# zendesk/min-tfs-client

Measured on AMD Instinct MI355X. Metric: predict_req_per_s, higher is better.
Workload: dtype fp32; 1 GPU; model=identity-echo[resnet50], global_batch=32, parallelism=dp1, pipeline=4, encoding=turbo, grpc_impl=native, copy_mode=1, streaming=auto, transport=unix, servers_per_rank=1, gpu=True

## Files before the change

### min_tfs_client_amd/ops/csrc/grpc_transport.cpp

```cpp
#include <pybind11/eval.h>
#include <pybind11/functional.h>
#include <pybind11/pybind11.h>
#include <pybind11/stl.h>
#include <torch/extension.h>

#include <c10/hip/HIPCachingAllocator.h>
#include <c10/hip/HIPGuard.h>
#include <c10/hip/HIPStream.h>

#include <algorithm>
#include <atomic>
#include <chrono>
#include <condition_variable>
#include <cstring>
#include <deque>
#include <map>
#include <memory>
#include <mutex>
#include <set>
#include <string>
#include <thread>
#include <unordered_map>
#include <vector>

#include "h2core.h"
#include "hpack.h"
#include "sharded.h"
#include "staging.h"
#include "wire.h"

namespace py = pybind11;

namespace {

using h2::Buf;
using h2::Conn;
using h2::ConnError;
using h2::FrameHeader;

struct WireRegion {
  size_t offset;
  size_t nbytes;
  uintptr_t ptr;
  bool device;
};

void write_message_with_regions(Conn& conn, uint32_t stream,
                                const uint8_t* buf, size_t len,
                                const std::vector<WireRegion>& regions,
                                bool end_stream) {
  h2::DataMessageWriter w(conn, stream, len, end_stream);
  size_t pos = 0;
  for (const auto& r : regions) {
    if (r.offset < pos || r.nbytes > len || r.offset > len - r.nbytes)
      throw ConnError("bad streaming region");
    if (r.offset > pos) w.write(buf + pos, r.offset - pos);
    if (!r.device) {
      w.write(reinterpret_cast<const uint8_t*>(r.ptr), r.nbytes);
    } else {
      mi355x_staging::Lease lease;
      lease.ctx->d2h(reinterpret_cast<const void*>(r.ptr), r.nbytes,
                     [&w](const void* chunk, size_t n) {
                       w.write(static_cast<const uint8_t*>(chunk), n);
                     });
    }
    pos = r.offset + r.nbytes;
  }
  if (pos < len) w.write(buf + pos, len - pos);
  w.finish();
}

bool extract_streaming_reply(py::handle result,
                             std::unique_ptr<py::buffer_info>* info,
                             const uint8_t** buf, size_t* len,
                             std::vector<WireRegion>* regions) {
  if (!py::hasattr(result, "_wire_regions")) return false;
  py::object buffer = result.attr("buffer");
  *info = std::make_unique<py::buffer_info>(py::buffer(buffer).request());
  *buf = static_cast<const uint8_t*>((*info)->ptr);
  *len = size_t((*info)->size) * size_t((*info)->itemsize);
  for (auto item : result.attr("_wire_regions")) {
    auto t = py::reinterpret_borrow<py::tuple>(item);
    regions->push_back(WireRegion{
        t[0].cast<size_t>(), t[1].cast<size_t>(),
        uintptr_t(t[2].cast<uint64_t>()), t[3].cast<bool>()});
  }
  return true;
}

struct RpcCallError : std::runtime_error {
  int code;
  RpcCallError(int code_, const std::string& msg)
      : std::runtime_error(msg), code(code_) {}
};

constexpr int GRPC_OK = 0;
constexpr int GRPC_CANCELLED = 1;
constexpr int GRPC_UNKNOWN = 2;
constexpr int GRPC_INVALID_ARGUMENT = 3;
constexpr int GRPC_DEADLINE_EXCEEDED = 4;
constexpr int GRPC_RESOURCE_EXHAUSTED = 8;
constexpr int GRPC_UNIMPLEMENTED = 12;
constexpr int GRPC_INTERNAL = 13;
constexpr int GRPC_UNAVAILABLE = 14;

struct OwnedBuf {
  Buf buf;
  explicit OwnedBuf(Buf&& b) : buf(std::move(b)) {}
};

class PinnedPool {
 public:
  static PinnedPool& instance() {
    static PinnedPool* pool = new PinnedPool();
    return *pool;
  }

  static constexpr size_t kMinPinned = 1u << 20;
  static constexpr size_t kMaxCached = 512u << 20;

  bool available() {
    int state = state_.load(std::memory_order_acquire);
    if (state == 0) {
      int n = 0;
      bool ok = hipGetDeviceCount(&n) == hipSuccess && n > 0;
      state = ok ? 1 : -1;
      state_.store(state, std::memory_order_release);
    }
    return state > 0;
  }

  uint8_t* get(size_t n, size_t* cap_out) {
    if (n < kMinPinned || !available()) return nullptr;
    size_t cap = size_class(n);
    {
      std::lock_guard<std::mutex> lk(mu_);
      auto& fl = free_[cap];
      if (!fl.empty()) {
        uint8_t* p = fl.back();
        fl.pop_back();
        cached_ -= cap;
        *cap_out = cap;
        return p;
      }
    }
    void* p = nullptr;
    if (hipHostMalloc(&p, cap) != hipSuccess) return nullptr;
    *cap_out = cap;
    return static_cast<uint8_t*>(p);
  }

  void put(uint8_t* p, size_t cap) {
    {
      std::lock_guard<std::mutex> lk(mu_);
      if (cached_ + cap <= kMaxCached) {
        free_[cap].push_back(p);
        cached_ += cap;
        return;
      }
    }
    (void)hipHostFree(p);
  }

  static void deleter(void* ctx, uint8_t* p, size_t cap) {
    static_cast<PinnedPool*>(ctx)->put(p, cap);
  }

 private:
  static size_t size_class(size_t n) {
    size_t cap = kMinPinned;
    while (cap < n) cap <<= 1;
    return cap;
  }
  std::atomic<int> state_{0};
  std::mutex mu_;
  std::map<size_t, std::vector<uint8_t*>> free_;
  size_t cached_ = 0;
};


inline bool tf_dtype_to_scalar(int dt, at::ScalarType* st) {
  switch (dt) {
    case 1: *st = at::kFloat; return true;
    case 2: *st = at::kDouble; return true;
    case 3: *st = at::kInt; return true;
    case 4: *st = at::kByte; return true;
    case 5: *st = at::kShort; return true;
    case 6: *st = at::kChar; return true;
    case 8: *st = at::kComplexFloat; return true;
    case 9: *st = at::kLong; return true;
    case 10: *st = at::kBool; return true;
    case 14: *st = at::kBFloat16; return true;
    case 17: *st = at::kUInt16; return true;
    case 18: *st = at::kComplexDouble; return true;
    case 19: *st = at::kHalf; return true;
    case 22: *st = at::kUInt32; return true;
    case 23: *st = at::kUInt64; return true;
    default: return false;
  }
}


inline void record_consumer_stream(
    std::vector<std::pair<std::string, at::Tensor>>& outs, int device) {
  if (outs.empty()) return;
  auto cur = c10::hip::getCurrentHIPStream(
      static_cast<c10::DeviceIndex>(device));
  for (auto& kv : outs)
    c10::hip::HIPCachingAllocator::recordStream(
        kv.second.storage().data_ptr(), cur);
}

struct MsgAssemblyFwd;

class ProspectStreams {
 public:
  static ProspectStreams& instance() {
    static ProspectStreams* p = new ProspectStreams();
    return *p;
  }

  static constexpr int kPerDevice = 4;

  hipStream_t get(int device) {
    std::lock_guard<std::mutex> lk(mu_);
    auto it = per_dev_.find(device);
    if (it == per_dev_.end()) {
      std::vector<hipStream_t> v;
      if (hipSetDevice(device) == hipSuccess) {
        for (int i = 0; i < kPerDevice; ++i) {
          hipStream_t s = nullptr;
          if (hipStreamCreateWithFlags(&s, hipStreamNonBlocking) !=
              hipSuccess)
            break;
          v.push_back(s);
        }
      }
      it = per_dev_.emplace(device, std::move(v)).first;
    }
    if (it->second.empty()) return nullptr;
    return it->second[rr_++ % it->second.size()];
  }

 private:
  std::mutex mu_;
  std::unordered_map<int, std::vector<hipStream_t>> per_dev_;
  size_t rr_ = 0;
};

struct DeviceParse {
  bool enabled = false;
  bool failed = false;
  bool done = false;
  int device = 0;
  hipStream_t stream = nullptr;
  int spec_field = 2;
  int map_field = 1;
  std::string spec_name, spec_signature, spec_label;
  int64_t spec_version = -1;
  std::vector<std::string> out_filter;
  std::function<bool(const std::string&)> skip_model;
  size_t pos = 0;
  int state = 0;
  size_t entry_end = 0, tp_end = 0;
  std::string cur_name;
  int cur_dtype = 0;
  std::vector<int64_t> cur_shape;
  bool cur_has_tensor = false;
  at::Tensor cur_tensor;
  bool in_content = false;
  size_t content_off = 0, content_len = 0, content_copied = 0;
  bool copies_issued = false;
  std::vector<std::pair<std::string, at::Tensor>> outs;

  static constexpr size_t kCopyBatch = 1u << 20;

  void fail() {
    failed = true;
    in_content = false;
  }

  void quiesce() {
    if (copies_issued && stream != nullptr) {
      (void)hipStreamSynchronize(stream);
      copies_issued = false;
    }
  }

  DeviceParse() = default;
  DeviceParse(const DeviceParse&) = delete;
  DeviceParse& operator=(const DeviceParse&) = delete;
  DeviceParse(DeviceParse&& o) noexcept { *this = std::move(o); }
  DeviceParse& operator=(DeviceParse&& o) noexcept {
    if (this != &o) {
      quiesce();
      enabled = o.enabled; failed = o.failed; done = o.done;
      device = o.device; stream = o.stream;
      spec_field = o.spec_field; map_field = o.map_field;
      spec_name = std::move(o.spec_name);
      spec_signature = std::move(o.spec_signature);
      spec_label = std::move(o.spec_label);
      spec_version = o.spec_version;
      out_filter = std::move(o.out_filter);
      skip_model = std::move(o.skip_model);
      pos = o.pos; state = o.state;
      entry_end = o.entry_end; tp_end = o.tp_end;
      cur_name = std::move(o.cur_name);
      cur_dtype = o.cur_dtype;
      cur_shape = std::move(o.cur_shape);
      cur_has_tensor = o.cur_has_tensor;
      cur_tensor = std::move(o.cur_tensor);
      in_content = o.in_content;
      content_off = o.content_off;
      content_len = o.content_len;
      content_copied = o.content_copied;
      copies_issued = o.copies_issued;
      outs = std::move(o.outs);
      o.copies_issued = false;
      o.enabled = false;
      o.stream = nullptr;
    }
    return *this;
  }
  ~DeviceParse() { quiesce(); }
};

struct MsgAssembly {
  uint8_t prefix[5];
  size_t prefix_have = 0;
  Buf msg;
  size_t msg_have = 0;
  bool have_len = false;

  void feed_from_socket(int fd, size_t n) {
    while (n > 0) {
      if (prefix_have < 5) {
        size_t take = 5 - prefix_have < n ? 5 - prefix_have : n;
        h2::read_full(fd, prefix + prefix_have, take);
        prefix_have += take;
        n -= take;
        if (prefix_have == 5) {
          if (prefix[0] != 0)
            throw RpcCallError(GRPC_UNIMPLEMENTED,
                               "compressed gRPC messages not supported");
          uint32_t len = h2::be32(prefix + 1);
          if (len > (1u << 30))
            throw RpcCallError(
                GRPC_RESOURCE_EXHAUSTED,
                "received message larger than max (" +
                    std::to_string(len) + " vs 1073741824)");
          size_t cap = 0;
          auto& pool = PinnedPool::instance();
          uint8_t* pinned = pool.get(len, &cap);
          if (pinned != nullptr)
            msg.adopt(pinned, cap, &PinnedPool::deleter, &pool);
          else
            msg.alloc(len);
          msg.len = len;
          have_len = true;
        }
        continue;
      }
      if (!have_len || msg_have + n > msg.len)
        throw ConnError("DATA overruns gRPC message length");
      h2::read_full(fd, msg.p + msg_have, n);
      msg_have += n;
      n = 0;
    }
  }

  bool complete() const { return have_len && msg_have == msg.len; }
};

inline void device_parse_advance(DeviceParse& dp, MsgAssembly& body) {
  if (!dp.enabled || dp.failed || dp.done) return;
  if (!body.have_len) return;
  if (dp.pos == 0 && dp.outs.empty() && !dp.in_content) {
    if (body.msg.deleter == nullptr || body.msg.len < (1u << 20)) {
      dp.enabled = false;
      return;
    }
  }
  const uint8_t* base = body.msg.p;
  const size_t watermark = body.msg_have;
  const size_t total = body.msg.len;

  auto issue_copies = [&]() -> bool {
    size_t span_end = dp.content_off + dp.content_len;
    size_t have_end = watermark < span_end ? watermark : span_end;
    size_t done_abs = dp.content_off + dp.content_copied;
    if (have_end > done_abs) {
      size_t n = have_end - done_abs;
      bool flush = have_end == span_end || body.complete();
      if (n >= DeviceParse::kCopyBatch || flush) {
        if (hipSetDevice(dp.device) != hipSuccess) { dp.fail(); return false; }
        char* dst = static_cast<char*>(dp.cur_tensor.data_ptr())
                    + dp.content_copied;
        if (hipMemcpyAsync(dst, base + done_abs, n, hipMemcpyHostToDevice,
                           dp.stream) != hipSuccess) {
          dp.fail();
          return false;
        }
        dp.copies_issued = true;
        dp.content_copied += n;
      }
    }
    return dp.content_copied == dp.content_len;
  };

  try {
    while (true) {
      if (dp.in_content) {
        if (!issue_copies()) return;
        if (dp.failed) return;
        dp.in_content = false;
        dp.pos = dp.content_off + dp.content_len;
        dp.cur_has_tensor = true;
      }
      tfswire::Cursor c{base + dp.pos, base + watermark};
      const uint8_t* step_start = c.p;
      try {
        if (dp.state == 0) {
          if (dp.pos == total) {
            dp.done = true;
            return;
          }
          int wt = 0;
          int f = c.read_tag(&wt);
          if (f == dp.spec_field && wt == tfswire::WT_LEN) {
            tfswire::Cursor spec = c.read_len_delim();
            while (!spec.done()) {
              int swt = 0;
              int sf = spec.read_tag(&swt);
              if (sf == 1 && swt == tfswire::WT_LEN) {
                tfswire::Cursor v = spec.read_len_delim();
                dp.spec_name.assign(reinterpret_cast<const char*>(v.p),
                                    size_t(v.end - v.p));
              } else if (sf == 2 && swt == tfswire::WT_LEN) {
                tfswire::Cursor v = spec.read_len_delim();
                while (!v.done()) {
                  int vwt = 0;
                  int vf = v.read_tag(&vwt);
                  if (vf == 1 && vwt == tfswire::WT_VARINT)
                    dp.spec_version = int64_t(v.read_varint());
                  else
                    v.skip(vwt);
                }
              } else if (sf == 3 && swt == tfswire::WT_LEN) {
                tfswire::Cursor v = spec.read_len_delim();
                dp.spec_signature.assign(
                    reinterpret_cast<const char*>(v.p),
                    size_t(v.end - v.p));
              } else if (sf == 4 && swt == tfswire::WT_LEN) {
                tfswire::Cursor v = spec.read_len_delim();
                dp.spec_label.assign(reinterpret_cast<const char*>(v.p),
                                     size_t(v.end - v.p));
              } else {
                spec.skip(swt);
              }
            }
            if (dp.skip_model && dp.skip_model(dp.spec_name)) {
              dp.enabled = false;
              return;
            }
            dp.pos = size_t(c.p - base);
          } else if (f == dp.map_field && wt == tfswire::WT_LEN) {
            uint64_t len = c.read_varint();
            size_t body_off = size_t(c.p - base);
            if (body_off + len > total) { dp.fail(); return; }
            dp.entry_end = body_off + len;
            dp.pos = body_off;
            dp.state = 1;
          } else if (dp.spec_field == 1 && f == 3 &&
                     wt == tfswire::WT_LEN) {
            tfswire::Cursor v = c.read_len_delim();
            dp.out_filter.emplace_back(
                reinterpret_cast<const char*>(v.p), size_t(v.end - v.p));
            dp.pos = size_t(c.p - base);
          } else {
            dp.fail();
            return;
          }
        } else if (dp.state == 1) {
          int wt = 0;
          int f = c.read_tag(&wt);
          if (f != 1 || wt != tfswire::WT_LEN) { dp.fail(); return; }
          tfswire::Cursor key = c.read_len_delim();
          dp.cur_name.assign(reinterpret_cast<const char*>(key.p),
                             size_t(key.end - key.p));
          f = c.read_tag(&wt);
          if (f != 2 || wt != tfswire::WT_LEN) { dp.fail(); return; }
          uint64_t len = c.read_varint();
          size_t body_off = size_t(c.p - base);
          if (body_off + len > dp.entry_end) { dp.fail(); return; }
          dp.tp_end = body_off + len;
          dp.pos = body_off;
          dp.state = 2;
          dp.cur_dtype = 0;
          dp.cur_shape.clear();
          dp.cur_has_tensor = false;
          dp.cur_tensor = at::Tensor();
        } else {
          if (dp.pos == dp.tp_end) {
            if (!dp.cur_has_tensor) {
              int64_t numel = 1;
              for (int64_t d : dp.cur_shape) numel *= d;
              at::ScalarType st;
              if (numel == 0 && tf_dtype_to_scalar(dp.cur_dtype, &st)) {
                c10::hip::HIPStreamGuard g(c10::hip::getStreamFromExternal(
                    dp.stream, static_cast<c10::DeviceIndex>(dp.device)));
                dp.cur_tensor = at::empty(
                    dp.cur_shape, at::TensorOptions().dtype(st).device(
                                      at::kCUDA, dp.device));
                dp.cur_has_tensor = true;
              } else {
                dp.fail();
                return;
              }
            }
            dp.outs.emplace_back(dp.cur_name, dp.cur_tensor);
            dp.cur_tensor = at::Tensor();
            if (dp.pos != dp.entry_end) { dp.fail(); return; }
            dp.state = 0;
            continue;
          }
          int wt = 0;
          int f = c.read_tag(&wt);
          if (f == 1 && wt == tfswire::WT_VARINT) {
            dp.cur_dtype = int(c.read_varint());
          } else if (f == 2 && wt == tfswire::WT_LEN) {
            tfswire::Cursor sh = c.read_len_delim();
            dp.cur_shape.clear();
            while (!sh.done()) {
              int swt = 0;
              int sf = sh.read_tag(&swt);
              if (sf == 2 && swt == tfswire::WT_LEN) {
                tfswire::Cursor dim = sh.read_len_delim();
                int64_t size = 0;
                while (!dim.done()) {
                  int dwt = 0;
                  int df = dim.read_tag(&dwt);
                  if (df == 1 && dwt == tfswire::WT_VARINT)
                    size = int64_t(dim.read_varint());
                  else
                    dim.skip(dwt);
                }
                dp.cur_shape.push_back(size);
              } else if (sf == 3) {
                dp.fail();
                return;
              } else {
                sh.skip(swt);
              }
            }
          } else if (f == 3 && wt == tfswire::WT_VARINT) {
            (void)c.read_varint();
          } else if (f == 4 && wt == tfswire::WT_LEN) {
            uint64_t len = c.read_varint();
            size_t off = size_t(c.p - base);
            if (off + len > dp.tp_end) { dp.fail(); return; }
            at::ScalarType st;
            if (!tf_dtype_to_scalar(dp.cur_dtype, &st)) { dp.fail(); return; }
            int64_t numel = 1;
            for (int64_t d : dp.cur_shape) numel *= d;
            size_t esize = at::elementSize(st);
            if (uint64_t(numel) * esize != len) { dp.fail(); return; }
            {
              c10::hip::HIPStreamGuard g(c10::hip::getStreamFromExternal(
                  dp.stream, static_cast<c10::DeviceIndex>(dp.device)));
              dp.cur_tensor = at::empty(
                  dp.cur_shape,
                  at::TensorOptions().dtype(st).device(at::kCUDA,
                                                       dp.device));
            }
            dp.content_off = off;
            dp.content_len = size_t(len);
            dp.content_copied = 0;
            dp.in_content = true;
            dp.pos = off;
            continue;
          } else {
            dp.fail();
            return;
          }
          dp.pos = size_t(c.p - base);
        }
      } catch (const std::exception&) {
        (void)step_start;
        if (body.complete()) dp.fail();
        return;
      }
    }
  } catch (...) {
    dp.fail();
  }
}

struct HeaderBlock {
  std::string block;
  bool end_stream = false;
  bool done = false;
};

inline void read_headers_fragment(int fd, const FrameHeader& fh,
                                  std::string* out) {
  uint32_t len = fh.length;
  uint8_t pad = 0;
  if (fh.flags & h2::FL_PADDED) {
    h2::read_full(fd, &pad, 1);
    if (len < 1u + pad) throw ConnError("bad padding");
    len -= 1;
  }
  if (fh.flags & h2::FL_PRIORITY) {
    uint8_t prio[5];
    if (len < 5) throw ConnError("bad priority");
    h2::read_full(fd, prio, 5);
    len -= 5;
  }
  len -= pad;
  size_t off = out->size();
  out->resize(off + len);
  h2::read_full(fd, reinterpret_cast<uint8_t*>(&(*out)[off]), len);
  if (pad) h2::discard(fd, pad);
}

inline const std::string* find_header(const std::vector<h2::Header>& hs,
                                      const char* name) {
  for (auto& h : hs)
    if (h.first == name) return &h.second;
  return nullptr;
}

inline std::string make_response_headers_block() {
  h2::HpackEncoder enc;
  std::string block;
  enc.add_indexed(&block, 8);
  enc.add_literal(&block, 31, "application/grpc");
  return block;
}

inline std::string make_trailers_block(int status, const std::string& msg) {
  h2::HpackEncoder enc;
  std::string block;
  enc.add_literal(&block, "grpc-status", std::to_string(status));
  if (!msg.empty())
    enc.add_literal(&block, "grpc-message", h2::percent_encode(msg));
  return block;
}

inline std::string make_trailers_only_block(int status,
                                            const std::string& msg) {
  h2::HpackEncoder enc;
  std::string block;
  enc.add_indexed(&block, 8);
  enc.add_literal(&block, 31, "application/grpc");
  enc.add_literal(&block, "grpc-status", std::to_string(status));
  if (!msg.empty())
    enc.add_literal(&block, "grpc-message", h2::percent_encode(msg));
  return block;
}

inline bool echo_eligible(const tfswire::ParsedPredict& req,
                          const std::map<std::string, std::set<int64_t>>&
                              models) {
  if (!req.output_filter.empty()) return false;
  auto it = models.find(req.model_spec.name);
  if (it == models.end()) return false;
  if (req.model_spec.version >= 0 &&
      it->second.find(req.model_spec.version) == it->second.end())
    return false;
  if (!req.model_spec.version_label.empty()) return false;
  for (auto& t : req.tensors)
    if (t.content == nullptr) return false;
  return true;
}

struct EchoResponse {
  Buf skeleton;
  std::vector<WireRegion> regions;
};

inline EchoResponse build_echo_response(const tfswire::ParsedPredict& req) {
  constexpr size_t kEchoMinRegion = 64 * 1024;
  std::vector<std::string> names;
  std::vector<tfswire::TensorMeta> metas;
  std::vector<const uint8_t*> payloads;
  names.reserve(req.tensors.size());
  for (auto& t : req.tensors) {
    std::string name = t.name;
    const std::string suffix = "_input";
    if (name.size() > suffix.size() &&
        name.compare(name.size() - suffix.size(), suffix.size(), suffix) ==
            0) {
      name = name.substr(0, name.size() - suffix.size()) + "_output";
    }
    names.push_back(std::move(name));
    metas.push_back({t.dtype, t.shape, t.content_bytes});
    payloads.push_back(t.content);
  }
  const std::string sig = req.model_spec.signature_name.empty()
                              ? "serving_default"
                              : req.model_spec.signature_name;
  auto plan = tfswire::plan_predict_message(false, req.model_spec.name,
                                            req.model_spec.version, sig,
                                            names, metas);
  EchoResponse r;
// ... 508 lines not shown
      std::lock_guard<std::mutex> lk(handler_mu_);
      parsed_path = parsed_paths_.count(t.path) != 0;
    }
    bool have_parse = parsed_path && t.dparse.enabled &&
                      !t.dparse.failed && t.dparse.done;
    t.dparse.quiesce();
    if (!Py_IsInitialized() || _Py_IsFinalizing()) {
      send_error_response(t, GRPC_UNAVAILABLE, "server shutting down");
      return;
    }
    int err_code = 0;
    std::string err_msg;
    py::object result;
    {
      py::gil_scoped_acquire gil;
      py::object fn;
      {
        std::lock_guard<std::mutex> lk(handler_mu_);
        auto it = py_handlers_.find(t.path);
        if (it != py_handlers_.end()) fn = it->second;
      }
      if (!fn) {
        err_code = GRPC_UNIMPLEMENTED;
        err_msg = "service method unregistered: " + t.path;
      } else
      try {
        py::memoryview view = py::memoryview::from_memory(
            t.msg.p, py::ssize_t(t.msg.len));
        if (parsed_path) {
          py::object spec = py::none();
          py::object outs = py::none();
          if (have_parse) {
            record_consumer_stream(t.dparse.outs, t.dparse.device);
            py::dict sd;
            sd["name"] = t.dparse.spec_name;
            sd["version"] = t.dparse.spec_version;
            sd["signature_name"] = t.dparse.spec_signature;
            sd["version_label"] = t.dparse.spec_label;
            py::list filt;
            for (auto& f2 : t.dparse.out_filter) filt.append(py::str(f2));
            sd["output_filter"] = filt;
            py::dict od;
            for (auto& kv : t.dparse.outs)
              od[py::str(kv.first)] = kv.second;
            spec = std::move(sd);
            outs = std::move(od);
          }
          result = fn(view, spec, outs);
        } else {
          result = fn(view);
        }
        t.dparse.outs.clear();
      } catch (py::error_already_set& e) {
        err_code = GRPC_UNKNOWN;
        try {
          py::object exc = e.value();
          if (py::hasattr(exc, "grpc_code"))
            err_code = exc.attr("grpc_code").cast<int>();
          if (py::hasattr(exc, "grpc_details"))
            err_msg = exc.attr("grpc_details").cast<std::string>();
          else
            err_msg = py::str(exc).cast<std::string>();
        } catch (...) {
          err_msg = "handler error";
        }
        e.restore();
        PyErr_Clear();
      }
    }
    if (err_code != 0) {
      send_error_response(t, err_code, err_msg);
      return;
    }
    std::unique_ptr<py::buffer_info> info;
    const uint8_t* ptr = nullptr;
    size_t len = 0;
    bool streaming = false;
    std::vector<WireRegion> regions;
    {
      py::gil_scoped_acquire gil;
      try {
        streaming = extract_streaming_reply(result, &info, &ptr, &len,
                                            &regions);
        if (!streaming) {
          info = std::make_unique<py::buffer_info>(
              py::buffer(result).request());
          ptr = static_cast<const uint8_t*>(info->ptr);
          len = size_t(info->size) * size_t(info->itemsize);
        }
      } catch (...) {
        info.reset();
        ptr = nullptr;
      }
    }
    if (!ptr) {
      send_error_response(t, GRPC_INTERNAL,
                          "handler returned a non-buffer object");
    } else {
      try {
        if (streaming) {
          t.conn->send_headers(t.stream, make_response_headers_block(),
                               false);
          write_message_with_regions(*t.conn, t.stream, ptr, len, regions,
                                     false);
          t.conn->send_headers(t.stream, make_trailers_block(GRPC_OK, ""),
                               true);
          t.conn->close_send_stream(t.stream);
        } else {
          send_ok_response(t, ptr, len);
        }
      } catch (...) {
        py::gil_scoped_acquire gil;
        info.reset();
        result = py::object();
        throw;
      }
    }
    py::gil_scoped_acquire gil;
    info.reset();
    result = py::object();
  }

  void send_ok_response(Task& t, const uint8_t* data, size_t n) {
    t.conn->send_headers(t.stream, make_response_headers_block(), false);
    t.conn->send_data_message(t.stream, data, n, false);
    t.conn->send_headers(t.stream, make_trailers_block(GRPC_OK, ""), true);
    t.conn->close_send_stream(t.stream);
  }

  void send_error_response(Task& t, int code, const std::string& msg) {
    t.conn->send_headers(t.stream, make_trailers_only_block(code, msg),
                         true);
    t.conn->close_send_stream(t.stream);
  }

  void stop_internal(bool wait) {
    bool was_running = running_.exchange(false);
    stopping_ = true;
    for (int fd : listen_fds_) {
      ::shutdown(fd, SHUT_RDWR);
      ::close(fd);
    }
    listen_fds_.clear();
    {
      std::lock_guard<std::mutex> lk(conns_mu_);
      for (auto& kv : conns_) kv.second->mark_broken("server stopping");
    }
    q_cv_.notify_all();
    if (!was_running && !wait) return;
    for (auto& th : accept_threads_)
      if (th.joinable()) th.join();
    accept_threads_.clear();
    {
      std::map<uint64_t, std::thread> threads;
      {
        std::lock_guard<std::mutex> lk(conns_mu_);
        threads.swap(conn_threads_);
      }
      for (auto& kv : threads)
        if (kv.second.joinable()) kv.second.join();
      std::lock_guard<std::mutex> lk(conns_mu_);
      conns_.clear();
      finished_conns_.clear();
    }
    for (auto& w : workers_)
      if (w.joinable()) w.join();
    workers_.clear();
    for (auto& up : unix_paths_) ::unlink(up.c_str());
    unix_paths_.clear();
    if (Py_IsInitialized()) {
      py::gil_scoped_acquire gil;
      py_handlers_.clear();
    }
  }
};


class GrpcChannel {
 public:
  explicit GrpcChannel(const std::string& target,
                       std::string authority = "")
      : authority_(std::move(authority)) {
    if (authority_.empty()) {
      authority_ = target.rfind("unix:", 0) == 0 ? "localhost" : target;
    }
    int fd = h2::connect_target(target);
    conn_ = std::make_shared<Conn>(fd);
    h2::write_all(fd, reinterpret_cast<const uint8_t*>(h2::kPreface),
                  h2::kPrefaceLen);
    conn_->send_initial_settings();
    reader_ = std::thread([this] { reader_loop(); });
  }

  ~GrpcChannel() { close(); }

  void close() {
    bool was = closed_.exchange(true);
    if (was) return;
    conn_->mark_broken("channel closed");
    if (reader_.joinable()) reader_.join();
    fail_all_pending(GRPC_UNAVAILABLE, "channel closed");
  }

  uint32_t begin_stream(const std::string& path, double timeout_s) {
    auto p = std::make_shared<Pending>();
    uint32_t id;
    {
      std::unique_lock<std::mutex> lk(mu_);
      cv_.wait(lk, [&] {
        int64_t maxs;
        {
          std::lock_guard<std::mutex> flk(conn_->fc_mu);
          maxs = conn_->peer_max_streams;
          if (conn_->broken) return true;
        }
        return maxs < 0 || int64_t(pending_.size()) < maxs;
      });
      {
        std::lock_guard<std::mutex> flk(conn_->fc_mu);
        if (conn_->broken)
          throw RpcCallError(GRPC_UNAVAILABLE,
                             "channel broken: " + conn_->broken_why);
      }
      id = next_stream_;
      next_stream_ += 2;
      streams_started_.fetch_add(1, std::memory_order_relaxed);
      pending_[id] = p;
      conn_->open_send_stream(id);
      std::string block = make_request_headers(path, timeout_s);
      try {
        conn_->send_headers(id, block, false);
      } catch (const std::exception& e) {
        pending_.erase(id);
        conn_->close_send_stream(id);
        throw RpcCallError(GRPC_UNAVAILABLE, e.what());
      }
    }
    return id;
  }

  uint32_t start_call(const std::string& path, const uint8_t* data,
                      size_t len, double timeout_s) {
    uint32_t id = begin_stream(path, timeout_s);
    try {
      conn_->send_data_message(id, data, len, true);
    } catch (const std::exception& e) {
      std::lock_guard<std::mutex> lk(mu_);
      pending_.erase(id);
      conn_->close_send_stream(id);
      throw RpcCallError(GRPC_UNAVAILABLE, e.what());
    }
    return id;
  }

  hipStream_t device_stream(int dev) {
    return ProspectStreams::instance().get(dev);
  }

  uint32_t start_call_streaming(const std::string& path, const uint8_t* buf,
                                size_t len,
                                const std::vector<WireRegion>& regions,
                                double timeout_s, int parse_device = -1) {
    uint32_t id = begin_stream(path, timeout_s);
    if (parse_device >= 0) {
      hipStream_t ds = device_stream(parse_device);
      if (ds != nullptr) {
        auto p = find_pending(id);
        if (p) {
          std::lock_guard<std::mutex> lk(p->m);
          p->dparse.enabled = true;
          p->dparse.device = parse_device;
          p->dparse.stream = ds;
        }
      }
    }
    try {
      write_message_with_regions(*conn_, id, buf, len, regions, true);
    } catch (const std::exception& e) {
      std::lock_guard<std::mutex> lk(mu_);
      pending_.erase(id);
      conn_->close_send_stream(id);
      throw RpcCallError(GRPC_UNAVAILABLE, e.what());
    }
    return id;
  }

  struct ParsedResult {
    Buf resp;
    bool parsed_ok = false;
    std::vector<std::pair<std::string, at::Tensor>> outs;
  };

  ParsedResult wait_parsed(uint32_t id, double timeout_s) {
    std::shared_ptr<Pending> p;
    {
      std::lock_guard<std::mutex> lk(mu_);
      auto it = pending_.find(id);
      if (it == pending_.end())
        throw RpcCallError(GRPC_INTERNAL, "unknown call handle");
      p = it->second;
    }
    auto quiesce = [&] {
      std::lock_guard<std::mutex> lk(p->m);
      if (p->dparse.enabled && p->dparse.stream != nullptr)
        (void)hipStreamSynchronize(p->dparse.stream);
    };
    std::unique_lock<std::mutex> lk(p->m);
    bool ok = true;
    if (timeout_s > 0) {
      ok = p->cv.wait_for(lk, std::chrono::duration<double>(timeout_s),
                          [&] { return p->done; });
    } else {
      p->cv.wait(lk, [&] { return p->done; });
    }
    if (!ok) {
      lk.unlock();
      quiesce();
      {
        std::lock_guard<std::mutex> glk(mu_);
        pending_.erase(id);
      }
      try {
        conn_->send_rst_stream(id, 8 );
      } catch (...) {
      }
      conn_->close_send_stream(id);
      cv_.notify_all();
      throw RpcCallError(GRPC_DEADLINE_EXCEEDED, "Deadline Exceeded");
    }
    ParsedResult r;
    r.resp = std::move(p->body.msg);
    int status = p->grpc_status;
    std::string msg = p->message;
    bool parsed = p->dparse.enabled && !p->dparse.failed && p->dparse.done;
    if (parsed) r.outs = std::move(p->dparse.outs);
    bool need_sync = p->dparse.enabled && p->dparse.stream != nullptr;
    hipStream_t ds = p->dparse.stream;
    lk.unlock();
    if (need_sync && hipStreamSynchronize(ds) != hipSuccess) parsed = false;
    if (parsed) record_consumer_stream(r.outs, r.outs.empty() ? 0 :
        r.outs.front().second.get_device());
    {
      std::lock_guard<std::mutex> glk(mu_);
      pending_.erase(id);
    }
    conn_->close_send_stream(id);
    cv_.notify_all();
    if (status != GRPC_OK)
      throw RpcCallError(status < 0 ? GRPC_INTERNAL : status, msg);
    r.parsed_ok = parsed;
    return r;
  }

  uint64_t streams_started() const {
    return streams_started_.load(std::memory_order_relaxed);
  }

  Buf wait(uint32_t id, double timeout_s) {
    std::shared_ptr<Pending> p;
    {
      std::lock_guard<std::mutex> lk(mu_);
      auto it = pending_.find(id);
      if (it == pending_.end())
        throw RpcCallError(GRPC_INTERNAL, "unknown call handle");
      p = it->second;
    }
    std::unique_lock<std::mutex> lk(p->m);
    bool ok = true;
    if (timeout_s > 0) {
      ok = p->cv.wait_for(lk, std::chrono::duration<double>(timeout_s),
                          [&] { return p->done; });
    } else {
      p->cv.wait(lk, [&] { return p->done; });
    }
    if (!ok) {
      lk.unlock();
      {
        std::lock_guard<std::mutex> glk(mu_);
        pending_.erase(id);
      }
      try {
        conn_->send_rst_stream(id, 8 );
      } catch (...) {
      }
      conn_->close_send_stream(id);
      cv_.notify_all();
      throw RpcCallError(GRPC_DEADLINE_EXCEEDED, "Deadline Exceeded");
    }
    Buf resp = std::move(p->body.msg);
    int status = p->grpc_status;
    std::string msg = p->message;
    lk.unlock();
    {
      std::lock_guard<std::mutex> glk(mu_);
      pending_.erase(id);
    }
    conn_->close_send_stream(id);
    cv_.notify_all();
    if (status != GRPC_OK)
      throw RpcCallError(status < 0 ? GRPC_INTERNAL : status, msg);
    return resp;
  }

 private:
  struct Pending {
    std::mutex m;
    std::condition_variable cv;
    bool done = false;
    int grpc_status = -1;
    std::string message;
    std::vector<h2::Header> resp_headers;
    HeaderBlock hb;
    MsgAssembly body;
    DeviceParse dparse;
  };

  std::shared_ptr<Conn> conn_;
  std::thread reader_;
  std::string authority_;
  std::atomic<bool> closed_{false};
  std::mutex mu_;
  std::condition_variable cv_;
  std::unordered_map<uint32_t, std::shared_ptr<Pending>> pending_;
  uint32_t next_stream_ = 1;
  std::atomic<uint64_t> streams_started_{0};

  std::string make_request_headers(const std::string& path,
                                   double timeout_s) {
    h2::HpackEncoder enc;
    std::string block;
    enc.add_indexed(&block, 3);
    enc.add_indexed(&block, 6);
    enc.add_literal(&block, 4, path, true);
    enc.add_literal(&block, 1, authority_);
    enc.add_literal(&block, "te", "trailers");
    enc.add_literal(&block, 31, "application/grpc");
    if (timeout_s > 0) {
      long ms = long(timeout_s * 1000.0);
      if (ms < 1) ms = 1;
      enc.add_literal(&block, "grpc-timeout", std::to_string(ms) + "m");
    }
    return block;
  }

  std::shared_ptr<Pending> find_pending(uint32_t id) {
    std::lock_guard<std::mutex> lk(mu_);
    auto it = pending_.find(id);
    return it == pending_.end() ? nullptr : it->second;
  }

  void complete(const std::shared_ptr<Pending>& p, int status,
                std::string msg) {
    {
      std::lock_guard<std::mutex> lk(p->m);
      if (p->done) return;
      p->grpc_status = status;
      p->message = std::move(msg);
      p->done = true;
    }
    p->cv.notify_all();
  }

  void fail_all_pending(int status, const std::string& msg) {
    std::vector<std::shared_ptr<Pending>> ps;
    {
      std::lock_guard<std::mutex> lk(mu_);
      for (auto& kv : pending_) ps.push_back(kv.second);
    }
    for (auto& p : ps) complete(p, status, msg);
    cv_.notify_all();
  }

  void process_headers(uint32_t stream, const std::shared_ptr<Pending>& p,
                       std::vector<h2::Header>&& headers, bool end_stream) {
    const std::string* gs = find_header(headers, "grpc-status");
    if (gs != nullptr || end_stream) {
      int status = GRPC_UNKNOWN;
      std::string msg = "missing grpc-status";
      if (gs) {
        status = std::atoi(gs->c_str());
        const std::string* gm = find_header(headers, "grpc-message");
        msg = gm ? h2::percent_decode(*gm) : "";
      }
      complete(p, status, std::move(msg));
    } else {
      std::lock_guard<std::mutex> lk(p->m);
      p->resp_headers = std::move(headers);
    }
  }

  void reader_loop() {
    h2::HpackDecoder decoder;
    uint32_t continuation_stream = 0;
    try {
      while (true) {
        FrameHeader fh = h2::read_frame_header(conn_->fd);
        switch (fh.type) {
          case h2::F_DATA: {
            auto p = find_pending(fh.stream);
            uint32_t len = fh.length;
            uint8_t pad = 0;
            if (fh.flags & h2::FL_PADDED) {
              h2::read_full(conn_->fd, &pad, 1);
              if (len < 1u + pad) throw ConnError("bad padding");
              len -= 1;
            }
            uint32_t body_len = len - pad;
            if (!p) {
              h2::discard(conn_->fd, len);
            } else {
              std::lock_guard<std::mutex> lk(p->m);
              p->body.feed_from_socket(conn_->fd, body_len);
              if (p->dparse.enabled)
                device_parse_advance(p->dparse, p->body);
              if (pad) h2::discard(conn_->fd, pad);
            }
            conn_->account_received(fh.length);
            if ((fh.flags & h2::FL_END_STREAM) && p)
              complete(p, GRPC_UNKNOWN, "stream ended without trailers");
            break;
          }
          case h2::F_HEADERS: {
            auto p = find_pending(fh.stream);
            HeaderBlock hb;
            std::string* block_dst = p ? &p->hb.block : &hb.block;
            {
              FrameHeader tmp = fh;
              read_headers_fragment(conn_->fd, tmp, block_dst);
            }
            bool end_stream = (fh.flags & h2::FL_END_STREAM) != 0;
            if (p) p->hb.end_stream = end_stream;
            if (fh.flags & h2::FL_END_HEADERS) {
              auto headers = decoder.decode(
                  reinterpret_cast<const uint8_t*>(block_dst->data()),
                  block_dst->size());
              block_dst->clear();
              if (p)
                process_headers(fh.stream, p, std::move(headers),
                                end_stream);
            } else {
              continuation_stream = fh.stream;
            }
            break;
          }
          case h2::F_CONTINUATION: {
            auto p = find_pending(continuation_stream);
            std::string scratch;
            std::string* block_dst = p ? &p->hb.block : &scratch;
            size_t off = block_dst->size();
            block_dst->resize(off + fh.length);
            h2::read_full(conn_->fd,
                          reinterpret_cast<uint8_t*>(&(*block_dst)[off]),
                          fh.length);
            if (fh.flags & h2::FL_END_HEADERS) {
              auto headers = decoder.decode(
                  reinterpret_cast<const uint8_t*>(block_dst->data()),
                  block_dst->size());
              block_dst->clear();
              if (p)
                process_headers(continuation_stream, p, std::move(headers),
                                p->hb.end_stream);
              continuation_stream = 0;
            }
            break;
          }
          case h2::F_SETTINGS: {
            if (fh.flags & h2::FL_ACK) {
              h2::discard(conn_->fd, fh.length);
            } else {
              std::vector<uint8_t> payload(fh.length);
              if (fh.length)
                h2::read_full(conn_->fd, payload.data(), fh.length);
              conn_->apply_peer_settings(payload.data(), fh.length);
              conn_->send_settings_ack();
            }
            break;
          }
          case h2::F_PING: {
            uint8_t opaque[8];
            if (fh.length != 8) throw ConnError("bad PING");
            h2::read_full(conn_->fd, opaque, 8);
            if (!(fh.flags & h2::FL_ACK)) conn_->send_ping_ack(opaque);
            break;
          }
          case h2::F_WINDOW_UPDATE: {
            uint8_t buf4[4];
            if (fh.length != 4) throw ConnError("bad WINDOW_UPDATE");
            h2::read_full(conn_->fd, buf4, 4);
            conn_->apply_window_update(fh.stream,
                                       h2::be32(buf4) & 0x7fffffff);
            break;
          }
          case h2::F_RST_STREAM: {
            uint8_t buf4[4];
            if (fh.length != 4) throw ConnError("bad RST_STREAM");
            h2::read_full(conn_->fd, buf4, 4);
            auto p = find_pending(fh.stream);
            if (p)
              complete(p, GRPC_UNAVAILABLE,
                       "stream reset by server (http2 code " +
                           std::to_string(h2::be32(buf4)) + ")");
            break;
          }
          case h2::F_GOAWAY:
          default:
            h2::discard(conn_->fd, fh.length);
            break;
        }
      }
    } catch (const std::exception& e) {
      conn_->mark_broken(e.what());
      fail_all_pending(GRPC_UNAVAILABLE,
                       std::string("connection lost: ") + e.what());
    }
  }
};


inline int scalar_to_tf_dtype(at::ScalarType t) {
  switch (t) {
    case at::kFloat: return 1;
    case at::kDouble: return 2;
    case at::kInt: return 3;
    case at::kByte: return 4;
    case at::kShort: return 5;
    case at::kChar: return 6;
    case at::kComplexFloat: return 8;
    case at::kLong: return 9;
    case at::kBool: return 10;
    case at::kBFloat16: return 14;
    case at::kUInt16: return 17;
    case at::kComplexDouble: return 18;
    case at::kHalf: return 19;
    case at::kUInt32: return 22;
    case at::kUInt64: return 23;
    default:
      throw std::invalid_argument("unsupported torch dtype for TensorProto");
  }
}

class SenderPool {
 public:
// ... 558 lines not shown
```

### min_tfs_client_amd/ops/csrc/staging.h

```cpp
#pragma once

#include <hip/hip_runtime_api.h>

#include <chrono>
#include <condition_variable>
#include <cstdint>
#include <cstdio>
#include <cstdlib>
#include <cstring>
#include <mutex>
#include <stdexcept>
#include <string>
#include <utility>
#include <vector>

namespace mi355x_staging {

#define MI355X_STAGING_CHECK(expr)                                       \
  do {                                                                   \
    hipError_t _e = (expr);                                              \
    if (_e != hipSuccess)                                                \
      throw std::runtime_error(std::string("HIP error in staging: ") +   \
                               hipGetErrorString(_e) + " at " #expr);    \
  } while (0)

inline size_t chunk_size() {
  static const size_t v = [] {
    const char* e = std::getenv("MI355X_STAGING_CHUNK");
    long long n = e ? std::atoll(e) : 0;
    if (n < (1 << 20) || n > (32 << 20)) n = 4 << 20;
    return size_t(n);
  }();
  return v;
}
constexpr int kMaxCtx = 8;

struct Ctx {
  hipStream_t stream = nullptr;
  void* buf[2] = {nullptr, nullptr};
  hipEvent_t evt[2] = {};
  hipEvent_t producer_evt = {};
  double acquire_ms = 0.0;

  void init() {
    MI355X_STAGING_CHECK(
        hipStreamCreateWithFlags(&stream, hipStreamNonBlocking));
    for (int i = 0; i < 2; ++i) {
      MI355X_STAGING_CHECK(hipHostMalloc(&buf[i], chunk_size()));
      MI355X_STAGING_CHECK(
          hipEventCreateWithFlags(&evt[i], hipEventDisableTiming));
    }
    MI355X_STAGING_CHECK(
        hipEventCreateWithFlags(&producer_evt, hipEventDisableTiming));
  }

  void wait_producer(hipStream_t producer) {
    MI355X_STAGING_CHECK(hipEventRecord(producer_evt, producer));
    MI355X_STAGING_CHECK(hipStreamWaitEvent(stream, producer_evt, 0));
  }

  template <typename Consume>
  void d2h(const void* src_dev, size_t nbytes, Consume&& consume) {
    const size_t kChunk = chunk_size();
    size_t nchunks = (nbytes + kChunk - 1) / kChunk;
    const char* trace_path = std::getenv("MI355X_STAGING_TRACE");
    std::vector<double> wait_ms, consume_ms;
    size_t issued = 0;
    for (size_t c = 0; c < (nchunks < 2 ? nchunks : 2); ++c) {
      size_t off = c * kChunk;
      size_t len = nbytes - off < kChunk ? nbytes - off : kChunk;
      MI355X_STAGING_CHECK(hipMemcpyAsync(
          buf[c & 1], static_cast<const char*>(src_dev) + off, len,
          hipMemcpyDeviceToHost, stream));
      MI355X_STAGING_CHECK(hipEventRecord(evt[c & 1], stream));
      ++issued;
    }
    for (size_t c = 0; c < nchunks; ++c) {
      size_t off = c * kChunk;
      size_t len = nbytes - off < kChunk ? nbytes - off : kChunk;
      std::chrono::steady_clock::time_point t0, t1, t2;
      if (trace_path) t0 = std::chrono::steady_clock::now();
      MI355X_STAGING_CHECK(hipEventSynchronize(evt[c & 1]));
      if (trace_path) t1 = std::chrono::steady_clock::now();
      consume(static_cast<const void*>(buf[c & 1]), len);
      if (trace_path) {
        t2 = std::chrono::steady_clock::now();
        wait_ms.push_back(
            std::chrono::duration<double, std::milli>(t1 - t0).count());
        consume_ms.push_back(
            std::chrono::duration<double, std::milli>(t2 - t1).count());
      }
      if (issued < nchunks) {
        size_t noff = issued * kChunk;
        size_t nlen = nbytes - noff < kChunk ? nbytes - noff : kChunk;
        MI355X_STAGING_CHECK(hipMemcpyAsync(
            buf[issued & 1], static_cast<const char*>(src_dev) + noff, nlen,
            hipMemcpyDeviceToHost, stream));
        MI355X_STAGING_CHECK(hipEventRecord(evt[issued & 1], stream));
        ++issued;
      }
    }
    if (trace_path && !wait_ms.empty()) {
      FILE* f = std::fopen(trace_path, "a");
      if (f) {
        std::fprintf(f, "{\"nbytes\": %zu, \"chunks\": %zu, "
                     "\"acquire_ms\": %.4f, \"wait_ms\": [",
                     nbytes, nchunks, acquire_ms);
        for (size_t i = 0; i < wait_ms.size(); ++i)
          std::fprintf(f, "%s%.4f", i ? "," : "", wait_ms[i]);
        std::fprintf(f, "], \"consume_ms\": [");
        for (size_t i = 0; i < consume_ms.size(); ++i)
          std::fprintf(f, "%s%.4f", i ? "," : "", consume_ms[i]);
        std::fprintf(f, "]}\n");
        std::fclose(f);
      }
    }
  }

  template <typename Produce>
  void h2d(void* dst_dev, size_t nbytes, Produce&& produce) {
    const size_t kChunk = chunk_size();
    size_t nchunks = (nbytes + kChunk - 1) / kChunk;
    for (size_t c = 0; c < nchunks; ++c) {
      size_t off = c * kChunk;
      size_t len = nbytes - off < kChunk ? nbytes - off : kChunk;
      if (c >= 2) MI355X_STAGING_CHECK(hipEventSynchronize(evt[c & 1]));
      produce(buf[c & 1], len);
      MI355X_STAGING_CHECK(hipMemcpyAsync(
          static_cast<char*>(dst_dev) + off, buf[c & 1], len,
          hipMemcpyHostToDevice, stream));
      MI355X_STAGING_CHECK(hipEventRecord(evt[c & 1], stream));
    }
    MI355X_STAGING_CHECK(hipStreamSynchronize(stream));
  }
};

class Pool {
 public:
  static Pool& instance() {
    static Pool pool;
    return pool;
  }

  Ctx* acquire() {
    std::unique_lock<std::mutex> lk(mu_);
    cv_.wait(lk, [this] { return !free_.empty() || created_ < kMaxCtx; });
    if (!free_.empty()) {
      Ctx* c = free_.back();
      free_.pop_back();
      return c;
    }
    ++created_;
    lk.unlock();
    auto* c = new Ctx();
    try {
      c->init();
    } catch (...) {
      delete c;
      std::lock_guard<std::mutex> lk2(mu_);
      --created_;
      cv_.notify_one();
      throw;
    }
    return c;
  }

  void release(Ctx* c) {
    {
      std::lock_guard<std::mutex> lk(mu_);
      free_.push_back(c);
    }
    cv_.notify_one();
  }

 private:
  std::mutex mu_;
  std::condition_variable cv_;
  std::vector<Ctx*> free_;
  int created_ = 0;
};

struct Lease {
  Ctx* ctx;
  Lease() {
    if (std::getenv("MI355X_STAGING_TRACE") == nullptr) {
      ctx = Pool::instance().acquire();
      return;
    }
    auto t0 = std::chrono::steady_clock::now();
    ctx = Pool::instance().acquire();
    ctx->acquire_ms = std::chrono::duration<double, std::milli>(
                          std::chrono::steady_clock::now() - t0)
                          .count();
  }
  ~Lease() { Pool::instance().release(ctx); }
  Lease(const Lease&) = delete;
  Lease& operator=(const Lease&) = delete;
};

}
```

Measured before the change: 911.8 req/s.

## Use ramped D2H chunk sizes and event-based waits for device parse copies

D2H staging now uses a chunk plan that starts with a small first chunk (256 KiB by default) and doubles up to the max chunk size. This lets the consumer start serializing sooner, shortening pipeline fill latency. Separately, device-parse H2D copies now record a pooled event and wait on that event rather than synchronizing the whole stream. The stream is shared round-robin, so the event avoids waiting on other calls' copies. The cost is more memcpy and event calls per transfer for the smaller early chunks.

```diff
diff --git a/min_tfs_client_amd/ops/csrc/chunk_plan.h b/min_tfs_client_amd/ops/csrc/chunk_plan.h
--- /dev/null
+++ b/min_tfs_client_amd/ops/csrc/chunk_plan.h
@@ -0,0 +1,32 @@
+#pragma once
+
+#include <cstddef>
+#include <vector>
+
+namespace mi355x_staging {
+
+constexpr size_t kChunkAlign = 256;
+
+inline std::vector<size_t> chunk_plan(size_t nbytes, size_t first,
+                                      size_t max_chunk) {
+  max_chunk = max_chunk / kChunkAlign * kChunkAlign;
+  if (max_chunk == 0) max_chunk = kChunkAlign;
+  if (first == 0 || first >= max_chunk) {
+    first = max_chunk;
+  } else {
+    first = (first + kChunkAlign - 1) / kChunkAlign * kChunkAlign;
+    if (first > max_chunk) first = max_chunk;
+  }
+  std::vector<size_t> lens;
+  size_t cur = first;
+  size_t left = nbytes;
+  while (left > 0) {
+    size_t len = left < cur ? left : cur;
+    lens.push_back(len);
+    left -= len;
+    cur = cur > max_chunk / 2 ? max_chunk : cur * 2;
+  }
+  return lens;
+}
+
+}
diff --git a/min_tfs_client_amd/ops/csrc/grpc_transport.cpp b/min_tfs_client_amd/ops/csrc/grpc_transport.cpp
--- a/min_tfs_client_amd/ops/csrc/grpc_transport.cpp
+++ b/min_tfs_client_amd/ops/csrc/grpc_transport.cpp
@@ -248,12 +248,47 @@
   size_t rr_ = 0;
 };
 
+class ParseEvents {
+ public:
+  static ParseEvents& instance() {
+    static ParseEvents* p = new ParseEvents();
+    return *p;
+  }
+
+  hipEvent_t get(int device) {
+    {
+      std::lock_guard<std::mutex> lk(mu_);
+      auto& v = free_[device];
+      if (!v.empty()) {
+        hipEvent_t e = v.back();
+        v.pop_back();
+        return e;
+      }
+    }
+    hipEvent_t e = nullptr;
+    if (hipEventCreateWithFlags(&e, hipEventDisableTiming) != hipSuccess)
+      return nullptr;
+    return e;
+  }
+
+  void put(int device, hipEvent_t e) {
+    std::lock_guard<std::mutex> lk(mu_);
+    free_[device].push_back(e);
+  }
+
+ private:
+  std::mutex mu_;
+  std::unordered_map<int, std::vector<hipEvent_t>> free_;
+};
+
 struct DeviceParse {
   bool enabled = false;
   bool failed = false;
   bool done = false;
   int device = 0;
   hipStream_t stream = nullptr;
+  hipEvent_t copies_evt = nullptr;
+  bool evt_current = false;
   int spec_field = 2;
   int map_field = 1;
   std::string spec_name, spec_signature, spec_label;
@@ -281,10 +316,31 @@
   }
 
   void quiesce() {
-    if (copies_issued && stream != nullptr) {
-      (void)hipStreamSynchronize(stream);
-      copies_issued = false;
-    }
+    (void)wait_copies();
+    copies_issued = false;
+  }
+
+  void copy_issued() {
+    copies_issued = true;
+    if (copies_evt == nullptr)
+      copies_evt = ParseEvents::instance().get(device);
+    evt_current = copies_evt != nullptr &&
+                  hipEventRecord(copies_evt, stream) == hipSuccess;
+  }
+
+  hipError_t wait_copies() const {
+    if (!copies_issued || stream == nullptr) return hipSuccess;
+    if (evt_current && hipEventSynchronize(copies_evt) == hipSuccess)
+      return hipSuccess;
+    return hipStreamSynchronize(stream);
+  }
+
+  void release_event() {
+    if (copies_evt != nullptr) {
+      ParseEvents::instance().put(device, copies_evt);
+      copies_evt = nullptr;
+    }
+    evt_current = false;
   }
 
   DeviceParse() = default;
@@ -294,8 +350,11 @@
   DeviceParse& operator=(DeviceParse&& o) noexcept {
     if (this != &o) {
       quiesce();
+      release_event();
       enabled = o.enabled; failed = o.failed; done = o.done;
       device = o.device; stream = o.stream;
+      copies_evt = o.copies_evt; evt_current = o.evt_current;
+      o.copies_evt = nullptr; o.evt_current = false;
       spec_field = o.spec_field; map_field = o.map_field;
       spec_name = std::move(o.spec_name);
       spec_signature = std::move(o.spec_signature);
@@ -322,7 +381,10 @@
     }
     return *this;
   }
-  ~DeviceParse() { quiesce(); }
+  ~DeviceParse() {
+    quiesce();
+    release_event();
+  }
 };
 
 struct MsgAssembly {
@@ -401,7 +463,7 @@
           dp.fail();
           return false;
         }
-        dp.copies_issued = true;
+        dp.copy_issued();
         dp.content_copied += n;
       }
     }
@@ -1516,8 +1578,7 @@
     }
     auto quiesce = [&] {
       std::lock_guard<std::mutex> lk(p->m);
-      if (p->dparse.enabled && p->dparse.stream != nullptr)
-        (void)hipStreamSynchronize(p->dparse.stream);
+      (void)p->dparse.wait_copies();
     };
     std::unique_lock<std::mutex> lk(p->m);
     bool ok = true;
@@ -1548,10 +1609,14 @@
     std::string msg = p->message;
     bool parsed = p->dparse.enabled && !p->dparse.failed && p->dparse.done;
     if (parsed) r.outs = std::move(p->dparse.outs);
-    bool need_sync = p->dparse.enabled && p->dparse.stream != nullptr;
+    bool need_sync = p->dparse.copies_issued && p->dparse.stream != nullptr;
     hipStream_t ds = p->dparse.stream;
+    hipEvent_t de = p->dparse.evt_current ? p->dparse.copies_evt : nullptr;
     lk.unlock();
-    if (need_sync && hipStreamSynchronize(ds) != hipSuccess) parsed = false;
+    if (need_sync &&
+        (de == nullptr || hipEventSynchronize(de) != hipSuccess) &&
+        hipStreamSynchronize(ds) != hipSuccess)
+      parsed = false;
     if (parsed) record_consumer_stream(r.outs, r.outs.empty() ? 0 :
         r.outs.front().second.get_device());
     {
diff --git a/min_tfs_client_amd/ops/csrc/staging.h b/min_tfs_client_amd/ops/csrc/staging.h
--- a/min_tfs_client_amd/ops/csrc/staging.h
+++ b/min_tfs_client_amd/ops/csrc/staging.h
@@ -14,6 +14,8 @@
 #include <utility>
 #include <vector>
 
+#include "chunk_plan.h"
+
 namespace mi355x_staging {
 
 #define MI355X_STAGING_CHECK(expr)                                       \
@@ -33,6 +35,15 @@
   }();
   return v;
 }
+inline size_t first_chunk_size() {
+  static const size_t v = [] {
+    const char* e = std::getenv("MI355X_STAGING_FIRST_CHUNK");
+    long long n = (e && *e) ? std::atoll(e) : (256 << 10);
+    if (n < 0) n = 256 << 10;
+    return size_t(n);
+  }();
+  return v;
+}
 constexpr int kMaxCtx = 8;
 
 struct Ctx {
@@ -61,28 +72,27 @@
 
   template <typename Consume>
   void d2h(const void* src_dev, size_t nbytes, Consume&& consume) {
-    const size_t kChunk = chunk_size();
-    size_t nchunks = (nbytes + kChunk - 1) / kChunk;
+    const std::vector<size_t> lens =
+        chunk_plan(nbytes, first_chunk_size(), chunk_size());
+    const size_t nchunks = lens.size();
     const char* trace_path = std::getenv("MI355X_STAGING_TRACE");
     std::vector<double> wait_ms, consume_ms;
-    size_t issued = 0;
-    for (size_t c = 0; c < (nchunks < 2 ? nchunks : 2); ++c) {
-      size_t off = c * kChunk;
-      size_t len = nbytes - off < kChunk ? nbytes - off : kChunk;
+    size_t issued = 0, issued_off = 0;
+    auto issue_next = [&] {
       MI355X_STAGING_CHECK(hipMemcpyAsync(
-          buf[c & 1], static_cast<const char*>(src_dev) + off, len,
-          hipMemcpyDeviceToHost, stream));
-      MI355X_STAGING_CHECK(hipEventRecord(evt[c & 1], stream));
+          buf[issued & 1], static_cast<const char*>(src_dev) + issued_off,
+          lens[issued], hipMemcpyDeviceToHost, stream));
+      MI355X_STAGING_CHECK(hipEventRecord(evt[issued & 1], stream));
+      issued_off += lens[issued];
       ++issued;
-    }
+    };
+    while (issued < nchunks && issued < 2) issue_next();
     for (size_t c = 0; c < nchunks; ++c) {
-      size_t off = c * kChunk;
-      size_t len = nbytes - off < kChunk ? nbytes - off : kChunk;
       std::chrono::steady_clock::time_point t0, t1, t2;
       if (trace_path) t0 = std::chrono::steady_clock::now();
       MI355X_STAGING_CHECK(hipEventSynchronize(evt[c & 1]));
       if (trace_path) t1 = std::chrono::steady_clock::now();
-      consume(static_cast<const void*>(buf[c & 1]), len);
+      consume(static_cast<const void*>(buf[c & 1]), lens[c]);
       if (trace_path) {
         t2 = std::chrono::steady_clock::now();
         wait_ms.push_back(
@@ -90,15 +100,7 @@
         consume_ms.push_back(
             std::chrono::duration<double, std::milli>(t2 - t1).count());
       }
-      if (issued < nchunks) {
-        size_t noff = issued * kChunk;
-        size_t nlen = nbytes - noff < kChunk ? nbytes - noff : kChunk;
-        MI355X_STAGING_CHECK(hipMemcpyAsync(
-            buf[issued & 1], static_cast<const char*>(src_dev) + noff, nlen,
-            hipMemcpyDeviceToHost, stream));
-        MI355X_STAGING_CHECK(hipEventRecord(evt[issued & 1], stream));
-        ++issued;
-      }
+      if (issued < nchunks) issue_next();
     }
     if (trace_path && !wait_ms.empty()) {
       FILE* f = std::fopen(trace_path, "a");
```

After: 854.5 req/s. 6.3% lower.
